# akofke/fountain

Hardware: AMD Instinct MI355X
Metric: Mrays/s (primary+secondary) at fixed spp (higher is better)
Workload: dtype f32; 1 GPU; config 5 scene: 2309 baked copies of rounded_cube = 10002588 triangles (19979703 BVH nodes, depth 29), 4096x4096 film, PathIntegrator(max_depth 5, rr 1.0), 1024^2 env-map light; one step = 16 spp over the whole film; tiles=65536, tiles_per_gpu=65536, pipeline=wavefront, sampler=indexed xoshiro256+, per_gpu_workload=copies=2309,res=4096,spp_per_gpu=16

## Files before the change

fountain_amd/csrc/ftn_device.h:

```cpp
#ifndef FTN_DEVICE_H
#define FTN_DEVICE_H

#include <hip/hip_runtime.h>
#include "ftn_math.h"
#include "../../include/fountain_hip.h"

namespace ftn {

#define FTN_DEV_NOINLINE __device__ inline

#define FTN_GS 3
enum : uint32_t { GF_KIND_SPHERE = 1u, GF_HAS_NORMALS = 2u, GF_HAS_UVS = 4u, GF_FLIP = 8u, GF_LEAF_END = 16u , GF_HAS_TANGENTS = 32u  };
enum : uint32_t { LK_POINT = 0, LK_DISTANT = 1, LK_INFINITE = 2, LK_AREA = 3 };

struct DSphere {
    float o2w[16], o2w_inv[16], w2o[16];
    float radius, z_min, z_max, theta_min, theta_max, phi_max;
    uint32_t reverse_orientation, _pad;
};

struct DLight {
    uint32_t kind; int32_t prim;
    float rgb[3];
    float v[3];
// ... 15 lines not shown

struct DScene {
    const float4* nodes; const float4* geom; const uint4* prim_info;
    uint32_t geom_stride, _pad_gs;
    const float* N; const float* UV;
    const float* T;
    const DSphere* spheres; const ftn_material* materials; const DLight* lights;
    uint32_t n_nodes, n_prims, n_lights, n_inf_lights, n_spheres, _pad;
    const uint32_t* inf_lights;
    const float4* fat;
    float root_lo[3], root_hi[3];
    uint32_t root_is_leaf, n_fat;
    const ftn_texture* textures; const ftn_material_textures* mtex; const DImage* images; const float4* texels;
    uint32_t n_textures;
    uint32_t material_types;
    uint32_t env_only, _pad2;
    DLight env0;
    const float4* srec;
    const float4* quad;
    uint32_t n_quads, quad_stack_bound;
    const uint4* oct; const float4* oct_xbox;
    uint32_t n_octs, oct_stack_bound;
    const uint4* quad64; const float4* quad64_xbox;
    uint32_t n_quad64, quad64_stack_bound;
    const unsigned char* prim_class;
};

struct DCamera {
    float c2w[16]; float r2c[16];
    float shutter_open, shutter_close, lens_radius, focal_dist;
    float dx_camera[3], dy_camera[3];
// ... 906 lines not shown
```

fountain_amd/csrc/ftn_gbuffer.hip:

```cpp
#include "ftn_wf_internal.h"
#include "ftn_texture.h"
#include "ftn_gbuffer.h"
#include <algorithm>
#include <cstring>

namespace ftn {

#define GB_MAX_PASS_THROUGH 4096u
struct GbParams {
    float w2c[16];
    float* out;
    float4 *spillA, *spillB, *spillC;
    float4* rec;
};

__device__ inline Rgb gb_albedo(const ftn_material& m) {
    const Rgb a(m.a[0], m.a[1], m.a[2]), b(m.b[0], m.b[1], m.b[2]);
    switch (m.type) {
        case FTN_MAT_MATTE: return clamp_positive(a);
        case FTN_MAT_MIRROR: return clamp_positive(a);
        case FTN_MAT_METAL: return fresnel_conductor(1.0f, Rgb(1.0f), a, b);
        case FTN_MAT_PLASTIC: return a + b;
        default: return clamp_positive(a) + clamp_positive(b);
    }
// ... 147 lines not shown

int wavefront_gbuffer(WavefrontState** state, const RenderParams& P, const std::vector<DTile>& tiles, const float w2c[16], float* d_out,
                      float4* spill_a, float4* spill_b, float4* spill_c, hipStream_t stream, double* trace_ms_out) {
    knobs_begin();
    { int rc0 = wf_state_init(state); if (rc0) return rc0; }
    WavefrontState* st = *state;
    const uint32_t n_slots = (uint32_t)tiles.size() * 256u;
    const uint32_t total_samples = P.last_sample - P.first_sample;
    if (n_slots == 0 || total_samples == 0) return FTN_OK;
    WfPassPlan plan;
    int rc = wf_plan_passes(st, P, tiles.size() * 256u, total_samples, false, &plan);
    if (rc) return rc;
    const uint32_t S = plan.samples;
    if ((rc = trace4_prepare(st, P.S))) return rc;
    WfBuffers W = st->W;
    W.br = nullptr; W.pd = nullptr; W.pd_md = 0; W.pd_occ = 0; W.drain_sig = nullptr; W.drain_seq = 0; W.serial = 0; W.rng_replay = 0; W.mis_any = 0;
    W.gen_blocks = knob("FTN_GEN_BLOCKS", 1);
    uint32_t valid = 0; for (const DTile& t : tiles) valid += (uint32_t)((t.x1 - t.x0) * (t.y1 - t.y0));
    W.valid_per_sample = valid;
    GbParams G;
    memcpy(G.w2c, w2c, sizeof(G.w2c)); G.out = d_out; G.spillA = spill_a; G.spillB = spill_b; G.spillC = spill_c; G.rec = st->pd;
    const bool spheres = P.S.n_spheres != 0, tex = P.S.n_textures != 0;
    const size_t lds = (size_t)P.stack_entries * 256 * sizeof(uint32_t);
    const unsigned blocks_per_cu = (unsigned)std::max<size_t>(1, std::min<size_t>(8, (size_t)(160 * 1024) / std::max<size_t>(lds, 1)));
    const unsigned trace_grid_max = (unsigned)st->n_cu * blocks_per_cu;
    double trace_ms = 0.0;
    for (uint32_t s0 = 0; s0 < total_samples; s0 += S) {
        const uint32_t Sp = std::min(S, total_samples - s0);
        W.n_slots = n_slots; W.samples = Sp; W.n_paths = Sp * n_slots; W.first_sample = P.first_sample + s0; W.seg_cap = (uint32_t)st->cap_paths;
        launch_wf_new_pass(W, P.stats, stream);
        launch_wf_generate(P, W, 0, stream);
// ... 36 lines not shown
```

fountain_amd/csrc/ftn_scene_host.cpp:

```cpp
#include "ftn_bvh_host.h"
#include "ftn_texture.h"

#include <chrono>
#include <cstdio>
#include <cstdlib>
#include <cstring>
#include <memory>

using namespace ftn;

static Aabb prim_bounds(const ftn_scene_desc* d, const ftn_prim& p) {
    Aabb b = aabb_empty();
    if (p.shape_kind == FTN_SHAPE_TRIANGLE) {
        for (int k = 0; k < 3; k++) { uint32_t v = d->tri_indices[3 * (size_t)p.shape_index + k]; aabb_join_point(b, V3(d->P[3 * v], d->P[3 * v + 1], d->P[3 * v + 2])); }
    } else {
        const ftn_sphere& s = d->spheres[p.shape_index];
        const float lo[3] = {-s.radius, -s.radius, s.z_min}, hi[3] = {s.radius, s.radius, s.z_max};
        for (int c = 0; c < 8; c++) {
            V3 q((c & 4) ? hi[0] : lo[0], (c & 2) ? hi[1] : lo[1], (c & 1) ? hi[2] : lo[2]);
            aabb_join_point(b, m4_point(s.object_to_world.m, q));
        }
    }
    return b;
}
// ... 133 lines not shown
    bool quad64_off = env_is("FTN_QUAD64", 0);
    bool oct_off = env_is("FTN_OCT", 0);
    bool srec_off = env_is("FTN_SREC", 0);
    bool geom_on = env_is("FTN_GEOM", 1);
    bool legacy_arrays_on = env_is("FTN_LEGACY_ARRAYS", 1);
    bool env_cells_off = env_is("FTN_ENV_CELLS", 0);
    bool no_coarse_cdf = getenv("FTN_NO_COARSE_CDF") != nullptr;
    bool want_fat() const { return trace4_off || quad_off || fat_on; }
};

struct Upload {
    const ftn_scene_desc* d; ftn_scene* sc; const HostScene& hs; const SceneKnobs& knobs; size_t np;
    std::vector<float4> geom; std::vector<uint4> info; std::vector<uint8_t> leaf_end;
    std::vector<ftn_material> mats; std::vector<DLight> lights; std::vector<uint32_t> inf;
    uint32_t n_fat = 0, n_quads = 0, quad_bound = 0, n_quad64 = 0, quad64_bound = 0, n_octs = 0, oct_bound = 0;
    bool geom_in_srec = false, has_tex = false;
    Upload(const ftn_scene_desc* d_, ftn_scene* sc_, const SceneKnobs& k) : d(d_), sc(sc_), hs(sc_->host), knobs(k), np(sc_->host.order.size()) {}
};

template <class T> static int held_table(std::vector<DevBuf<T>>& held, const T* src, size_t n, const T** p) {
    held.emplace_back();
    const int rc = held.back().upload(src, n);
    *p = held.back().p;
    return rc;
}

static int node_records(const Upload& U, std::vector<float4>* out) {
    const HostScene& hs = U.hs;
    std::vector<float4>& nodes = *out;
    nodes.resize(2 * hs.nodes.size());
    parallel_for(hs.nodes.size(), [&](size_t i0, size_t i1) { for (size_t i = i0; i < i1; i++) {
// ... 148 lines not shown
    }
    if ((rc = sc->spheres.upload(sph.data(), sph.size()))) return rc;
    U.mats.assign(d->materials, d->materials + d->n_materials);
    U.has_tex = d->n_textures != 0 && d->textures != nullptr;
    for (size_t i = 0; i < U.mats.size(); i++) {
        bool textured = false;
        if (U.has_tex && d->material_textures) { const ftn_material_textures& mt = d->material_textures[i]; textured = (mt.a & mt.b & mt.s0 & mt.s1 & mt.s2) >= 0; }
        if (!textured) material_finalize(U.mats[i]);
    }
    return sc->materials.upload(U.mats.data(), U.mats.size());
}

static int prim_classes(Upload& U) {
    std::vector<unsigned char> cls(U.np);
    for (size_t i = 0; i < U.np; i++) { const int m = (int)U.info[2 * i].x; cls[i] = (unsigned char)(m < 0 || (size_t)m >= U.mats.size() ? 7u : std::min<uint32_t>(2u + U.mats[(size_t)m].type, 7u)); }
    return U.sc->prim_class.upload(cls.data(), cls.size());
}

struct EnvTables { std::vector<float4> tex4; std::vector<float> img, ccdf, cint, mcdf; uint32_t nu = 0, nv = 0; };

static void env_distribution(const ftn_envmap& e, DLight& L, EnvTables* T) {
    const uint32_t height = e.width, width = e.height;
    T->tex4.resize((size_t)e.width * e.height);
    for (size_t k = 0; k < T->tex4.size(); k++) T->tex4[k] = make_float4(e.texels[3 * k], e.texels[3 * k + 1], e.texels[3 * k + 2], 0.0f);
    DLight hostL = L; hostL.texels = T->tex4.data();
    std::vector<float>& img = T->img;
    img.resize((size_t)width * height);
    for (uint32_t j = 0; j < height; j++) {
        float v = (float)j / (float)height;
        float sin_theta = ftn_det::sinf_det(FTN_PI * ((float)j + 0.5f) / (float)height);
// ... 91 lines not shown
        if (L.kind == LK_INFINITE) {
            U.inf.push_back((uint32_t)l);
            if ((rc = env_light_tables(U, src, L))) return rc;
        }
    }
    if ((rc = U.sc->lights.upload(lights.data(), lights.size()))) return rc;
    return U.sc->inf_lights.upload(U.inf.data(), U.inf.size());
}

static void fill_dscene(Upload& U) {
    ftn_scene* sc = U.sc; const HostScene& hs = U.hs;
    DScene& D = sc->d; memset(&D, 0, sizeof(D));
    D.nodes = sc->nodes.p; D.geom = U.geom_in_srec ? sc->srec.p : sc->geom.p; D.geom_stride = U.geom_in_srec ? 8u : (uint32_t)FTN_GS; D.prim_info = sc->prim_info.p; D.N = sc->N.p; D.UV = sc->UV.p; D.T = sc->T.p; D.spheres = sc->spheres.p;
    D.materials = sc->materials.p; D.lights = sc->lights.p; D.inf_lights = sc->inf_lights.p;
    D.n_nodes = (uint32_t)hs.nodes.size(); D.n_prims = (uint32_t)U.np; D.n_lights = (uint32_t)U.lights.size(); D.n_inf_lights = (uint32_t)U.inf.size(); D.n_spheres = U.d->n_spheres;
    D.srec = sc->srec.p; D.prim_class = sc->prim_class.p;
    D.quad = sc->quad.p; D.n_quads = U.n_quads; D.quad_stack_bound = U.quad_bound;
    D.oct = sc->oct.p; D.oct_xbox = sc->oct_xbox.p; D.n_octs = U.n_octs; D.oct_stack_bound = U.oct_bound;
    D.quad64 = sc->quad64.p; D.quad64_xbox = sc->quad64_xbox.p; D.n_quad64 = U.n_quad64; D.quad64_stack_bound = U.quad64_bound;
    D.fat = sc->fat.p; D.n_fat = U.n_fat; D.root_is_leaf = (!hs.nodes.empty() && hs.nodes[0].is_leaf) ? 1u : 0u;
    for (int k = 0; k < 3; k++) { D.root_lo[k] = hs.nodes.empty() ? 0.0f : hs.nodes[0].bmin[k]; D.root_hi[k] = hs.nodes.empty() ? 0.0f : hs.nodes[0].bmax[k]; }
    if (U.lights.size() == 1 && U.lights[0].kind == LK_INFINITE) { D.env_only = 1; D.env0 = U.lights[0]; }
    sc->stack_entries = std::max<uint32_t>(hs.max_depth, 1u);
    for (const ftn_material& m : U.mats) if (m.type < 32u) D.material_types |= 1u << m.type;
}

static int textures_and_pyramids(Upload& U) {
    const ftn_scene_desc* d = U.d; ftn_scene* sc = U.sc;
    if (!U.has_tex) return FTN_OK;
    const int nt = (int)d->n_textures, ni = d->images ? (int)d->n_images : 0;
    std::vector<ftn_material_textures> mt(d->n_materials);
// ... 122 lines not shown
```

fountain_amd/csrc/ftn_wavefront.hip:

```cpp
#include "ftn_wf_internal.h"
#include "ftn_texture.h"
#include <string>
#include <cstdlib>
#include <hipcub/hipcub.hpp>

namespace ftn {

__global__ void __launch_bounds__(256) k_wf_generate(RenderParams P, WfBuffers W, int write_state) {
    const uint32_t i = blockIdx.x * 256u + threadIdx.x;
    if (i >= W.n_paths) return;
    const uint32_t slot = i / W.samples, s = i % W.samples;
    const DTile tile = P.tiles[slot >> 8];
    const int px = tile.x0 + (int)(slot & 15u), py = tile.y0 + (int)((slot >> 4) & 15u);
    if (px < tile.x1 && py < tile.y1) {
        Rng rng; rng.seed(indexed_key(P.seed, px, py, W.first_sample + s));
        V2 j = rng.next2();
        V2 p_film((float)px + j.x, (float)py + j.y);
        V2 p_lens = rng.next2();
        float time_u = rng.next();
        DRay ray = camera_ray(P.C, p_film, p_lens, time_u);
        W.ray[2 * (size_t)(i)] = make_float4(ray.o.x, ray.o.y, ray.o.z, 0.0f);
        W.ray[2 * (size_t)(i) + 1] = make_float4(ray.d.x, ray.d.y, ray.d.z, ray.t_max);
        if (write_state) {
            W.beta[i] = make_float4(1.0f, 1.0f, 1.0f, __uint_as_float(PS_ALIVE));
// ... 234 lines not shown
        uint32_t* T = &W.counters[CTR(13) + 4 * ((policy >> 8) & 7u)];
        atomicMax(&T[0], ~t_start); atomicMax(&T[1], ~t_dry); atomicMax(&T[2], t_dry); atomicMax(&T[3], (uint32_t)wall_clock64());
    }
#endif
    if (blockIdx.x == 0 && threadIdx.x == 0) atomicAdd(&stats->rays_any, (unsigned long long)count);
}

#define WF_NCLASS 8
__device__ inline uint32_t wf_class_of(const RenderParams& P, const WfBuffers& W, uint32_t entry) {
    if (entry & WF_Q_FIN) return 0u;
    const int prim = W.hit_prim[entry & WF_Q_ID_MASK];
    if (prim < 0 || (entry & WF_Q_DEPTH)) return 1u;
    return P.S.prim_class[prim];
}
#define WF_CLS_ROUNDS 32
__global__ void __launch_bounds__(256) k_wf_classify(RenderParams P, WfBuffers W, int in_q) {
    __shared__ unsigned char s_cls[WF_CLS_ROUNDS][256];
    __shared__ uint32_t s_cnt[WF_CLS_ROUNDS][WF_NCLASS][4];
    __shared__ uint32_t s_pre[WF_CLS_ROUNDS][WF_NCLASS];
    __shared__ uint32_t s_base[WF_NCLASS];
    const uint32_t count = W.counters[CTR(in_q == 0 ? 0 : 1)];
    const uint32_t stride = gridDim.x * 256u, rounds = (count + stride - 1) / stride;
    const uint32_t wave = threadIdx.x >> 6, lane = lane_id();
    for (uint32_t r0 = 0; r0 < rounds; r0 += WF_CLS_ROUNDS) {
        const uint32_t nr = rounds - r0 < WF_CLS_ROUNDS ? rounds - r0 : WF_CLS_ROUNDS;
        for (uint32_t r = 0; r < nr; r++) {
            const uint32_t qi = (r0 + r) * stride + blockIdx.x * 256u + threadIdx.x;
            uint32_t c = WF_NCLASS;
            if (qi < count) c = wf_class_of(P, W, W.q_active[in_q][qi]);
            s_cls[r][threadIdx.x] = (unsigned char)c;
#pragma unroll
            for (int k = 0; k < WF_NCLASS; k++) {
                const unsigned long long m = __ballot(c == (uint32_t)k);
                if (lane == 0) s_cnt[r][k][wave] = (uint32_t)__popcll(m);
            }
        }
        __syncthreads();
        if (threadIdx.x < WF_NCLASS) {
            const uint32_t k = threadIdx.x; uint32_t tot = 0;
            for (uint32_t r = 0; r < nr; r++) { s_pre[r][k] = tot; tot += s_cnt[r][k][0] + s_cnt[r][k][1] + s_cnt[r][k][2] + s_cnt[r][k][3]; }
            s_base[k] = tot ? atomicAdd(&W.cls[CTR(k)], tot) : 0u;
        }
        __syncthreads();
        for (uint32_t r = 0; r < nr; r++) {
// ... 12 lines not shown
    }
}

#ifndef FTN_SHADE_MIN_WAVES
#define FTN_SHADE_MIN_WAVES 1
#endif
#ifndef FTN_SHADE_WAVES_NOBSDF
#define FTN_SHADE_WAVES_NOBSDF 4
#endif
#ifndef FTN_SHADE_WAVES_MATTE
#define FTN_SHADE_WAVES_MATTE 3
#endif
#ifndef FTN_SHADE_WAVES_OTHER
#define FTN_SHADE_WAVES_OTHER 3
#endif
template <bool TEX, int MT, bool ENV>
__global__ void __launch_bounds__(256, (MT == -1 ? FTN_SHADE_MIN_WAVES : (MT == -2 ? FTN_SHADE_WAVES_NOBSDF : (MT == 0 ? FTN_SHADE_WAVES_MATTE : FTN_SHADE_WAVES_OTHER)))) k_wf_shade(RenderParams P, WfBuffers W, int in_q, uint32_t class_mask, uint32_t first ) {
    const DScene& S = P.S;
    uint32_t cbase[WF_NCLASS + 1], ccnt[WF_NCLASS];
    cbase[0] = 0;
#pragma unroll
    for (int k = 0; k < WF_NCLASS; k++) { ccnt[k] = ((class_mask >> k) & 1u) ? W.cls[CTR(k)] : 0u; cbase[k + 1] = cbase[k] + ((ccnt[k] + 255u) & ~255u); }
    const uint32_t count = cbase[WF_NCLASS];
    uint32_t* out_q = W.q_active[in_q ^ 1];
    uint32_t* out_count = &W.counters[CTR(in_q == 0 ? 1 : 0)];
    int err = 0;
    const uint32_t stride = gridDim.x * 256u;
    const uint32_t rounds = (count + stride - 1) / stride;
    for (uint32_t round = 0; round < rounds; round++) {
        const uint32_t qi = round * stride + blockIdx.x * 256u + threadIdx.x;
// ... 6 lines not shown
            have = qi - cb < cc;
            sorted_idx = c * W.seg_cap + (qi - cb);
        }
        bool push_active = false, push_closest = false, push_mis = false, push_shadow = false, push_mis_any = false;
        uint32_t p = 0, active_entry = 0;
        if (have) {
            p = W.q_sorted[sorted_idx];
            float4 bq = make_float4(1.0f, 1.0f, 1.0f, __uint_as_float(PS_ALIVE)), lq = make_float4(0.0f, 0.0f, 0.0f, 0.0f);
            if (!first) { if (W.br) { bq = W.br[2 * (size_t)p]; lq = W.br[2 * (size_t)p + 1]; } else { bq = W.beta[p]; lq = W.rad[p]; } }
            Rgb beta(bq.x, bq.y, bq.z), L(lq.x, lq.y, lq.z);
            uint32_t ps = __float_as_uint(bq.w);
            if (ps & PS_DIRECT) {
                float4 q0, q1, q2, q3 = make_float4(0.0f, 0.0f, 0.0f, 0.0f);
                if (W.pd) { const float4* Q = W.pd + 4 * (size_t)p; q0 = Q[0]; q1 = Q[1]; q2 = Q[2]; if (W.pd_md) q3 = Q[3]; } else { q0 = W.pend0[p]; q1 = W.pend1[p]; q2 = W.pend2[p]; }
                const uint32_t occ_word = __float_as_uint(q3.w);
                Rgb radiance(0.0f);
                if ((ps & PS_SHADOW) && !(W.pd_occ ? (occ_word & 0xffu) != 0u : W.occluded[p] != 0)) radiance = radiance + Rgb(q0.x, q0.y, q0.z);
                if (ps & PS_MIS_ANY) {
                    const int light_index = (int)__float_as_uint(lq.w);
                    const DLight& Lt = ENV ? S.env0 : S.lights[light_index];
                    const float4 md = W.pd_md ? q3 : W.ray[2 * (size_t)(p + W.n_paths) + 1];
                    Rgb inc(0.0f);
                    if (!(W.pd_occ ? (occ_word & 0xff00u) != 0u : W.occluded[p + W.n_paths] != 0)) inc = light_Le_env(Lt, V3(md.x, md.y, md.z));
                    if (!inc.is_black()) radiance = radiance + Rgb(q1.x, q1.y, q1.z) * inc * q0.w / q1.w;
                } else if (ps & PS_MIS) {
                    const int light_index = (int)__float_as_uint(lq.w);
                    const DLight& Lt = ENV ? S.env0 : S.lights[light_index];
                    const DHit mh = load_hit(W, p + W.n_paths);
                    const float4 mo = W.ray[2 * (size_t)(p + W.n_paths)], md = W.ray[2 * (size_t)(p + W.n_paths) + 1];
                    Rgb inc(0.0f);
                    if (mh.prim >= 0) {
                      if (!ENV) {
                        int h_mat, h_light; prim_mat_light(S, mh.prim, &h_mat, &h_light);
                        if (h_light >= 0 && h_light == light_index) {
                            DRay r0; r0.o = V3(mo.x, mo.y, mo.z); r0.d = V3(md.x, md.y, md.z); r0.t_max = FTN_INF; r0.time = 0.0f;
                            DSI s2; make_interaction(S, mh, r0, &s2);
                            inc = area_Le(Lt, s2.hit.n, -r0.d);
                        }
                      }
                    } else if (ENV || Lt.kind == LK_INFINITE) inc = light_Le_env(Lt, V3(md.x, md.y, md.z));
                    if (!inc.is_black()) radiance = radiance + Rgb(q1.x, q1.y, q1.z) * inc * q0.w / q1.w;
                }
                Rgb direct = Rgb(q2.x, q2.y, q2.z) * ((float)S.n_lights * radiance);
                L = L + direct;
                ps &= ~(PS_DIRECT | PS_SHADOW | PS_MIS | PS_MIS_ANY);
            }
            if (!(ps & PS_ALIVE)) {
                W.rad[p] = make_float4(L.r, L.g, L.b, 0.0f);
            } else {
                DRay ray0; ray0.o = V3(0.0f, 0.0f, 0.0f); ray0.d = V3(0.0f, 0.0f, 1.0f); ray0.t_max = FTN_INF; ray0.time = 0.0f;
                DHit h; h.t = FTN_INF; h.b0 = 0.0f; h.b1 = 0.0f; h.b2 = 0.0f; h.prim = -1;
                bool need_ray = true;
                if (MT == -2 && !first) { h.prim = W.hit_prim[p]; need_ray = h.prim >= 0 || (ps & PS_BOUNCE_MASK) == 0u || (ps & PS_SPECULAR) != 0u; }
                if (need_ray) {
                    const float4 ro = W.ray[2 * (size_t)(p)], rdv = W.ray[2 * (size_t)(p) + 1];
                    ray0.o = V3(ro.x, ro.y, ro.z); ray0.d = V3(rdv.x, rdv.y, rdv.z); ray0.t_max = rdv.w;
                    h = load_hit(W, p);
                }
                const bool hit = h.prim >= 0;
                uint32_t bounces = ps & PS_BOUNCE_MASK;
                const bool specular_bounce = (ps & PS_SPECULAR) != 0;
                DSI si;
                if (hit) make_interaction(S, h, ray0, &si);
                if (bounces == 0 || specular_bounce) {
                    if (hit) {
                        Rgb e(0.0f);
                        if (!ENV && si.light >= 0) e = area_Le(S.lights[si.light], si.hit.n, -ray0.d);
                        L = L + beta * e;
                    } else L = L + beta * (ENV ? Rgb(0.0f) + light_Le_env(S.env0, ray0.d) : scene_env_Le(S, ray0.d));
                }
                bool alive = true;
                uint32_t light_word = 0;
                if (!hit || bounces >= P.max_depth) alive = false;
                else {
                    Rng rng;
                    if (first) {
                        const uint32_t slot = p / W.samples, sidx = p % W.samples;
                        const DTile tile = P.tiles[slot >> 8];
                        rng.seed(indexed_key(P.seed, tile.x0 + (int)(slot & 15u), tile.y0 + (int)((slot >> 4) & 15u), W.first_sample + sidx));
                        (void)rng.next2(); (void)rng.next2(); (void)rng.next();
                    } else if (W.rng_replay) {
                        const uint32_t slot = p / W.samples, sidx = p % W.samples;
                        const DTile tile = P.tiles[slot >> 8];
                        rng.seed(indexed_key(P.seed, tile.x0 + (int)(slot & 15u), tile.y0 + (int)((slot >> 4) & 15u), W.first_sample + sidx));
// ... 92 lines not shown
                                    float q = fmax_(0.05f, 1.0f - beta.max_component());
                                    n_draws += 1u;
                                    if (rng.next() < q) alive = false; else beta = beta / (1.0f - q);
                                }
                                if (alive) {
                                    W.ray[2 * (size_t)(p)] = make_float4(nr.o.x, nr.o.y, nr.o.z, 0.0f); W.ray[2 * (size_t)(p) + 1] = make_float4(nr.d.x, nr.d.y, nr.d.z, nr.t_max);
                                    bounces += 1; push_closest = true;
                                }
                            } else alive = false;
                        }
                    }
                    if (W.rng_replay) ps = (ps & ((1u << PS_DRAWS_SHIFT) - 1u)) | (n_draws << PS_DRAWS_SHIFT);
                    else if (alive || W.serial) { W.rng01[p] = make_ulonglong2(rng.s0, rng.s1); W.rng23[p] = make_ulonglong2(rng.s2, rng.s3); }
                }
                ps = (ps & ~(PS_BOUNCE_MASK | PS_ALIVE)) | (bounces & PS_BOUNCE_MASK) | (alive ? PS_ALIVE : 0u);
                push_active = alive || (ps & PS_DIRECT);
                if (W.br) {
                    if (push_active) { W.br[2 * (size_t)p] = make_float4(beta.r, beta.g, beta.b, __uint_as_float(ps)); W.br[2 * (size_t)p + 1] = make_float4(L.r, L.g, L.b, __uint_as_float(light_word)); }
                    else W.rad[p] = make_float4(L.r, L.g, L.b, 0.0f);
                } else {
                    if (push_active) W.beta[p] = make_float4(beta.r, beta.g, beta.b, __uint_as_float(ps));
                    W.rad[p] = make_float4(L.r, L.g, L.b, __uint_as_float(light_word));
                }
                active_entry = p | (alive ? (bounces >= P.max_depth ? WF_Q_DEPTH : 0u) : WF_Q_FIN);
            }
            if (W.serial && !push_active) W.ser_retired[p] = 1;
        }
        {
            const bool pred[6] = {push_active, push_closest, push_mis, push_shadow, push_mis_any, push_mis_any};
            const uint32_t val[6] = {active_entry, p, p | WF_MIS_BIT, p, p | WF_MIS_BIT, 0u};
            uint32_t* const qs[6] = {out_q, W.q_closest, W.q_closest, W.q_shadow, W.q_shadow, nullptr};
            uint32_t* const cs[6] = {out_count, &W.counters[CTR(2)], &W.counters[CTR(2)], &W.counters[CTR(3)], &W.counters[CTR(3)], &W.counters[CTR(10)]};
            block_push<6>(pred, val, qs, cs);
// ... 259 lines not shown
        stats->camera_samples += (unsigned long long)W.samples * W.valid_per_sample;
    } else if (mode == 1) {
        W.counters[CTR(2)] = 0; W.counters[CTR(3)] = 0; W.counters[CTR(in_q == 0 ? 1 : 0)] = 0; W.counters[CTR(11)] = 0;
        for (int i = 16; i < 32; i++) W.counters[CTR(i)] = 0;
        for (int i = 32; i < 56; i++) W.counters[CTR(i)] = 0;
    } else if (mode == 2) {
        for (int i = 0; i < WF_NCLASS; i++) W.cls[CTR(i)] = 0;
    } else if (mode == 3) {
        for (int i = 0; i < 64; i++) W.counters[CTR(i)] = 0;
    }
}

#define WF_ACC_CHUNK 8u
__global__ void __launch_bounds__(256) k_wf_accumulate(RenderParams P, WfBuffers W) {
    __shared__ float4 s_rad[256 * WF_ACC_CHUNK];
    const uint32_t slot = blockIdx.x * 256u + threadIdx.x;
    uint32_t spill = 0, bc = 0, cam = 0; int err = 0;
    const FilmSlot fs = film_slot(P, W.n_slots, slot);
    const bool valid = fs.valid, in_crop = fs.in_crop; const int px = fs.px, py = fs.py; const size_t ai = fs.ai;
    float4 acc = make_float4(0.0f, 0.0f, 0.0f, 0.0f);
    if (in_crop) acc = P.accA[ai];
    const size_t block_first = (size_t)blockIdx.x * 256u * W.samples;
    for (uint32_t s0 = 0; s0 < W.samples; s0 += WF_ACC_CHUNK) {
        const uint32_t n = W.samples - s0 < WF_ACC_CHUNK ? W.samples - s0 : WF_ACC_CHUNK;
        for (uint32_t e = threadIdx.x; e < 256u * n; e += 256u) {
            const uint32_t sl = e / n, k = e - sl * n;
            const size_t p = block_first + (size_t)sl * W.samples + s0 + k;
            if (p < W.n_paths) s_rad[sl * WF_ACC_CHUNK + k] = W.rad[p];
        }
        __syncthreads();
        if (valid) {
            for (uint32_t k = 0; k < n; k++) {
                const float4 l = s_rad[threadIdx.x * WF_ACC_CHUNK + k];
                Rgb L(l.x, l.y, l.z);
                if (L.has_nans()) err = FTN_ERR_NAN_RADIANCE;
                Rng crng; crng.seed(indexed_key(P.seed, px, py, W.first_sample + s0 + k));
                const V2 j = crng.next2();
                if (film_add(fs.F, P.accA, P.accB, P.accC, V2((float)px + j.x, (float)py + j.y), L, in_crop ? px : FTN_OWN_NONE, py, &acc, &bc) != 1) spill++;
                cam++;
            }
        }
        __syncthreads();
    }
// ... 365 lines not shown
    if (rc) { wf_free(st); return rc; }
    const bool tex = P.S.n_textures != 0;
    if (n_tiles > st->ser_paths || (tex && !st->ser_tex)) {
        for (void*& m : st->ser_mem) { if (m) (void)hipFree(m); m = nullptr; }
        st->ser_paths = 0;
        WF_TRY(hipMalloc(&st->ser_mem[0], (size_t)n_tiles * sizeof(uint2)));
        WF_TRY(hipMalloc(&st->ser_mem[1], (size_t)n_tiles * sizeof(float2)));
        WF_TRY(hipMalloc(&st->ser_mem[2], (size_t)n_tiles));
        if (tex) WF_TRY(hipMalloc(&st->ser_mem[3], 3 * (size_t)n_tiles * sizeof(float4)));
        st->ser_paths = n_tiles; st->ser_tex = tex;
    }
    if ((rc = trace4_prepare(st, P.S))) return rc;
    WfBuffers W = st->W;
    W.serial = 1; W.ser_cursor = (uint2*)st->ser_mem[0]; W.ser_pfilm = (float2*)st->ser_mem[1]; W.ser_retired = (unsigned char*)st->ser_mem[2]; W.dfd = (float4*)st->ser_mem[3];
    W.n_slots = 0; W.samples = 1; W.n_paths = n_tiles; W.first_sample = 0; W.seg_cap = (uint32_t)st->cap_paths; W.valid_per_sample = 0;
    W.gen_blocks = 0; W.rng_replay = 0; W.br = nullptr; W.pd = nullptr; W.pd_md = 0; W.pd_occ = 0;
    const int count_mode = count ? (count_production ? 2 : 1) : 0;
    W.mis_any = ((!count || count_production) && knob("FTN_MIS_ANY", 1)) ? 1u : 0u;
    const bool spheres = P.S.n_spheres != 0;
    const size_t lds = (size_t)P.stack_entries * 256 * sizeof(uint32_t);
    const unsigned blocks_per_cu = (unsigned)std::max<size_t>(1, std::min<size_t>(8, (size_t)(160 * 1024) / std::max<size_t>(lds, 1)));
    const unsigned tg = std::min<unsigned>((unsigned)st->n_cu * blocks_per_cu, (2 * n_tiles + 255) / 256);
    const dim3 pgrid((n_tiles + 255) / 256), sgrid(std::min<unsigned>((unsigned)st->n_cu * 8u, (n_tiles + 255) / 256));
    const bool env = P.S.env_only && knob("FTN_SHADE_ENV", 1);
    hipEvent_t e0 = st->ev[0], e1 = st->ev[1];
    (void)hipEventRecord(e0, stream);
    hipLaunchKernelGGL(k_wf_reset, dim3(1), dim3(64), 0, stream, W, 3, 0, P.stats);
    if (tex) hipLaunchKernelGGL((k_wf_serial_advance<true>), pgrid, dim3(256), 0, stream, P, W, 0, 1); else hipLaunchKernelGGL((k_wf_serial_advance<false>), pgrid, dim3(256), 0, stream, P, W, 0, 1);
    int in_q = 0; unsigned long long rounds = 0, trace_launches = 0;
    if (!st->ser_host) WF_TRY(hipHostMalloc((void**)&st->ser_host, 2 * 16 * 32 * sizeof(uint32_t)));
    int polled_q[2] = {0, 0}; uint32_t* last = st->ser_host;
    const bool side_ok = st->side != nullptr && knob("FTN_WF_OVERLAP", 2) != 0 && getenv("ROCPROF_COUNTER_COLLECTION") == nullptr;
    const uint64_t max_rounds = 256u * (uint64_t)std::max<uint32_t>(P.spp, 1u) * ((uint64_t)P.max_depth + 4u + (1u << 12));
    for (uint64_t it = 0; it < max_rounds; it++) {
        const bool beside = it > 0 && side_ok;
        if (beside) { WF_TRY(hipEventRecord(st->ev_ready, stream)); WF_TRY(hipStreamWaitEvent(st->side, st->ev_ready, 0));
                      launch_trace(st, true, count_mode, spheres, tg, lds, st->side, P, W, W.q_shadow, &W.counters[CTR(3)], &W.counters[CTR(24)], 2 * n_tiles);
                      WF_TRY(hipEventRecord(st->ev_side, st->side)); }
        launch_trace(st, false, count_mode, spheres, tg, lds, stream, P, W, W.q_closest, &W.counters[CTR(2)], &W.counters[CTR(16)], 2 * n_tiles);
        trace_launches++;
        if (it > 0 && !beside) launch_trace(st, true, count_mode, spheres, tg, lds, stream, P, W, W.q_shadow, &W.counters[CTR(3)], &W.counters[CTR(24)], 2 * n_tiles);
        if (beside) WF_TRY(hipStreamWaitEvent(stream, st->ev_side, 0));
        hipLaunchKernelGGL(k_wf_reset, dim3(1), dim3(64), 0, stream, W, 2, in_q, P.stats);
        hipLaunchKernelGGL(k_wf_classify, sgrid, dim3(256), 0, stream, P, W, in_q);
        hipLaunchKernelGGL(k_wf_reset, dim3(1), dim3(64), 0, stream, W, 1, in_q, P.stats);
#define FTN_SH2(T, M, E, mask) hipLaunchKernelGGL((k_wf_shade<T, M, E>), sgrid, dim3(256), 0, stream, P, W, in_q, mask, 0u)
#define FTN_SH(M, mask) do { if (tex) { if (env) FTN_SH2(true, M, true, mask); else FTN_SH2(true, M, false, mask); } \
                             else { if (env) FTN_SH2(false, M, true, mask); else FTN_SH2(false, M, false, mask); } } while (0)
        if (!knob("FTN_SHADE_SPECIALISE", 1)) FTN_SH(-1, 0xffu);
        else {
            FTN_SH(-2, 0x83u);
            if (P.S.material_types & 1u) FTN_SH(0, 1u << 2);
            if (P.S.material_types & 2u) FTN_SH(1, 1u << 3);
            if (P.S.material_types & 4u) FTN_SH(2, 1u << 4);
            if (P.S.material_types & 8u) FTN_SH(3, 1u << 5);
            if (P.S.material_types & 16u) FTN_SH(4, 1u << 6);
        }
#undef FTN_SH2
#undef FTN_SH
// ... 50 lines not shown
    if ((rc = trace4_prepare(st, P.S))) return rc;
    if (dl_mode) { st->W.dlA = (float4*)st->dl_mem[0]; st->W.dlB = (float4*)st->dl_mem[1]; st->W.whT = (float4*)st->dl_mem[2]; st->W.dfd = (float4*)st->dl_mem[7]; }
    WfBuffers W = st->W;
    if (dl_mode) { W.sh = (float4*)st->dl_mem[3]; W.occluded = (unsigned char*)st->dl_mem[4]; W.q_shadow = (uint32_t*)st->dl_mem[5]; W.q_exc_any = (uint32_t*)st->dl_mem[6]; }
    if (!knob("FTN_ENV_CELLS_USE", 1)) P.S.env0.cells = nullptr;
    const bool spheres = P.S.n_spheres != 0;
    uint32_t valid = 0; for (const DTile& t : tiles) valid += (uint32_t)((t.x1 - t.x0) * (t.y1 - t.y0));
    W.valid_per_sample = valid;
    W.mis_any = ((!count || count_production) && knob("FTN_MIS_ANY", 1)) ? 1u : 0u;
    W.rng_replay = (!dl_mode && 5u + 8u * ((uint32_t)P.max_depth + 1u) <= 511u && knob("FTN_RNG_REPLAY", 1)) ? 1u : 0u;
    W.br = (!dl_mode && knob("FTN_WF_BR", 1)) ? st->br : nullptr;
    W.pd = (!dl_mode && knob("FTN_WF_PD", 3)) ? st->pd : nullptr;
    W.pd_md = (W.pd && knob("FTN_WF_PD", 3) >= 2) ? 1u : 0u;
    W.pd_occ = (W.pd && knob("FTN_WF_PD", 3) >= 3) ? 1u : 0u;
    W.gen_blocks = knob("FTN_GEN_BLOCKS", 1);
    const size_t lds = (size_t)P.stack_entries * 256 * sizeof(uint32_t);
    const unsigned blocks_per_cu = (unsigned)std::max<size_t>(1, std::min<size_t>(8, (size_t)(160 * 1024) / std::max<size_t>(lds, 1)));
    const unsigned trace_grid_max = (unsigned)st->n_cu * blocks_per_cu;
    const unsigned shade_grid_max = (unsigned)st->n_cu * 8u;
    double trace_ms = 0.0; unsigned long long trace_launches = 0, mis_any_rays = 0;
    double group_ms[4] = {0.0, 0.0, 0.0, 0.0}; unsigned long long group_n[4] = {0, 0, 0, 0};
    const uint32_t overlap_mode = knob("FTN_WF_OVERLAP", 2);
    const bool drain_gate = knob("FTN_WF_DRAIN_GATE", 1) != 0 && getenv("ROCPROF_COUNTER_COLLECTION") == nullptr;
    const uint32_t sort_bits = knob("FTN_WF_SORT", 0) ? std::min<uint32_t>(std::max<uint32_t>(knob("FTN_WF_SORT_BITS", 7), 1u), 9u) : 0u;
    uint32_t n_active = 0;
    int ev_used = 0;
    struct Span { int a, b, kind; };
    std::vector<Span> spans;
    static const char* const kGroup[4] = {"closest-hit trace", "any-hit trace", "classify + shade", "queue sort"};
    auto flush_events = [&]() -> int {
// ... 44 lines not shown
            trace_launches++;
            if (beside) WF_TRY(hipStreamWaitEvent(st->side, st->ev_ready, 0));
            if (gated) WF_TRY(hipStreamWaitValue32(st->side, st->drain_sig, W.drain_seq, hipStreamWaitValueGte, 0xffffffffu));
            if (it > 0) {
                const unsigned sg = std::min<unsigned>(trace_grid_max, (2 * W.n_paths + 255) / 256);
                hipStream_t as = beside ? st->side : stream;
                const int e = span_begin(as);
                launch_trace(st, true, count_mode, spheres, sg, lds, as, P, W, q_sh, &W.counters[CTR(3)], &W.counters[CTR(24)], 2 * W.n_paths, it == 1 && W.samples >= 4u);
                span_end(e, 1, as);
                if (beside) WF_TRY(hipEventRecord(st->ev_side, st->side));
            }
            {
                const int e_cls = span_begin(stream);
                const unsigned cg = std::min<unsigned>(shade_grid_max, (W.n_paths + 255) / 256);
                hipLaunchKernelGGL(k_wf_reset, dim3(1), dim3(64), 0, stream, W, 2, in_q, P.stats);
                hipLaunchKernelGGL(k_wf_classify, dim3(cg), dim3(256), 0, stream, P, W, in_q);
                span_end(e_cls, 2, stream);
            }
            if (beside) WF_TRY(hipStreamWaitEvent(stream, st->ev_side, 0));
            const int e_shade = span_begin(stream);
            hipLaunchKernelGGL(k_wf_reset, dim3(1), dim3(64), 0, stream, W, 1, in_q, P.stats);
            {
                const dim3 sgrid(std::min<unsigned>(shade_grid_max, (W.n_paths + 255) / 256));
                const bool tex = P.S.n_textures != 0;
                const uint32_t first = it == 0 ? 1u : 0u;
                if (dl_mode) {
                    if (whitted) { if (tex) hipLaunchKernelGGL((k_wf_shade_dl<true, true>), sgrid, dim3(256), 0, stream, P, W, in_q); else hipLaunchKernelGGL((k_wf_shade_dl<true, false>), sgrid, dim3(256), 0, stream, P, W, in_q); }
                    else { if (tex) hipLaunchKernelGGL((k_wf_shade_dl<false, true>), sgrid, dim3(256), 0, stream, P, W, in_q); else hipLaunchKernelGGL((k_wf_shade_dl<false, false>), sgrid, dim3(256), 0, stream, P, W, in_q); }
                } else if (!knob("FTN_SHADE_SPECIALISE", 1)) {
                    if (tex) hipLaunchKernelGGL((k_wf_shade<true, -1, false>), sgrid, dim3(256), 0, stream, P, W, in_q, 0xffu, first);
                    else hipLaunchKernelGGL((k_wf_shade<false, -1, false>), sgrid, dim3(256), 0, stream, P, W, in_q, 0xffu, first);
                } else {
                    const bool env = P.S.env_only && knob("FTN_SHADE_ENV", 1);
                    const unsigned grid_k = knob("FTN_SHADE_GRID", 0), grid_k_nb = knob("FTN_SHADE_GRID_NOBSDF", 0);
#define FTN_SH2(T, M, E, mask) do { const unsigned per_cu = (M) == -2 ? (grid_k_nb ? grid_k_nb : 2u * shade_wgs_per_cu<T, M, E>()) : (grid_k ? grid_k : shade_wgs_per_cu<T, M, E>()); \
                                    hipLaunchKernelGGL((k_wf_shade<T, M, E>), dim3(std::min<unsigned>((unsigned)st->n_cu * per_cu, (W.n_paths + 255) / 256)), dim3(256), 0, stream, P, W, in_q, mask, first); } while (0)
#define FTN_SH(M, mask) do { if (tex) { if (env) FTN_SH2(true, M, true, mask); else FTN_SH2(true, M, false, mask); } \
                             else { if (env) FTN_SH2(false, M, true, mask); else FTN_SH2(false, M, false, mask); } } while (0)
                    FTN_SH(-2, 0x83u);
                    if (P.S.material_types & 1u) FTN_SH(0, 1u << 2);
                    if (P.S.material_types & 2u) FTN_SH(1, 1u << 3);
                    if (P.S.material_types & 4u) FTN_SH(2, 1u << 4);
                    if (P.S.material_types & 8u) FTN_SH(3, 1u << 5);
                    if (P.S.material_types & 16u) FTN_SH(4, 1u << 6);
#undef FTN_SH2
#undef FTN_SH
                }
            }
            span_end(e_shade, 2, stream);
            in_q ^= 1;
            if (sort_bits) {
                WF_TRY(hipMemcpyAsync(st->host_counters, W.counters, 16 * 32 * sizeof(uint32_t), hipMemcpyDeviceToHost, stream));
                WF_TRY(hipStreamSynchronize(stream));
                polled = true;
// ... 7 lines not shown
                const int e_sort = span_begin(stream);
                if ((rc = sort_ray_queue(st, P, W, false, W.q_closest, st->host_counters[CTR(2)], W.q_sorted, k_in, k_out, sort_bits, stream, &q_cl))) return rc;
                if (knob("FTN_WF_SORT_ANY", 0) && (rc = sort_ray_queue(st, P, W, true, W.q_shadow, st->host_counters[CTR(3)], W.q_sorted + 2 * n, k_in, k_out, sort_bits, stream, &q_sh))) return rc;
                span_end(e_sort, 3, stream);
            }
            if (it >= P.max_depth || polled) {
                if (!polled) {
                    WF_TRY(hipMemcpyAsync(st->host_counters, W.counters, 16 * 32 * sizeof(uint32_t), hipMemcpyDeviceToHost, stream));
                    WF_TRY(hipStreamSynchronize(stream));
                }
                if (it >= P.max_depth && count && knob("FTN_WF_DEBUG", 0)) fprintf(stderr, "[wf] wave steps so far: node %u leaf %u; lanes during node steps (x64): idle %u waiting-with-leaf %u\n", st->host_counters[CTR(6)], st->host_counters[CTR(7)], st->host_counters[CTR(8)], st->host_counters[CTR(9)]);
                n_active = st->host_counters[CTR(in_q == 0 ? 0 : 1)];
                if (n_active == 0) break;
            }
        }
        if (W.mis_any) mis_any_rays += st->host_counters[CTR(10)];
        hipLaunchKernelGGL(k_wf_accumulate, dim3((n_slots + 255) / 256), dim3(256), 0, stream, P, W);
        if (hook) hook(hook_ctx, P, W, stream);
    }
    return FTN_OK;
    };
    rc = render_passes();
    { const int rc_flush = flush_events(); if (!rc) rc = rc_flush; }
    if (rc) return rc;
    WF_TRY(hipGetLastError());
    if (times) {
        times->trace_ms = trace_ms; times->trace_launches = trace_launches; times->mis_any_rays = mis_any_rays;
        times->any_ms = group_ms[1]; times->any_launches = group_n[1]; times->shade_ms = group_ms[2]; times->shade_launches = group_n[2]; times->sort_ms = group_ms[3];
    }
    return FTN_OK;
// ... 4 lines not shown
```

fountain_amd/csrc/ftn_wf_common.h:

```cpp
#ifndef FTN_WF_COMMON_H
#define FTN_WF_COMMON_H
#include "ftn_wavefront.h"
#include "ftn_film.h"

namespace ftn {

enum : uint32_t { PS_BOUNCE_MASK = 0xffffu, PS_SPECULAR = 1u << 16, PS_ALIVE = 1u << 17, PS_DIRECT = 1u << 18, PS_SHADOW = 1u << 19, PS_MIS = 1u << 20, PS_DELTA = 1u << 21, PS_MIS_ANY = 1u << 22  };
#define PS_DRAWS_SHIFT 23
#define WF_MIS_BIT 0x80000000u

struct WfBuffers {
    uint32_t n_paths;
    uint32_t n_slots;
    uint32_t samples;
    uint32_t first_sample;
    float4 *ray;
    float4* hit;
    int* hit_prim;
    float4 *sh;
    unsigned char* occluded;
    float4 *beta;
    float4 *rad;
    float4* br;
    ulonglong2 *rng01, *rng23;
// ... 5 lines not shown
    uint32_t* cls;
    uint32_t seg_cap;
    uint32_t* counters;
    uint32_t valid_per_sample;
    uint32_t* drain_sig; uint32_t drain_seq, drain_at;
    uint32_t *q_exc_closest, *q_exc_any;
    float4 *dlA, *dlB, *whT;
    float4* dfd;
    uint32_t serial;
    uint2* ser_cursor;
    float2* ser_pfilm;
    unsigned char* ser_retired;
    uint32_t rng_replay;
    uint32_t gen_blocks;
    uint32_t mis_any;
};

#define WF_Q_FIN 0x80000000u
#define WF_Q_DEPTH 0x40000000u
#define WF_Q_ID_MASK 0x0fffffffu

#define CTR(i) ((i) * 32)
__device__ inline uint32_t lane_id() { return threadIdx.x & 63u; }
__device__ inline void wave_push(bool pred, uint32_t value, uint32_t* queue, uint32_t* counter) {
    const unsigned long long m = __ballot(pred);
    if (m == 0) return;
    const int leader = __ffsll((long long)m) - 1;
    uint32_t base = 0;
    if ((int)lane_id() == leader) base = atomicAdd(counter, (uint32_t)__popcll(m));
    base = __shfl(base, leader, 64);
// ... 121 lines not shown
```

Baseline: 3234 Mrays/s.

## Defer direct-light and escape finishing to accumulate kernel in env-only wavefront

In env-only scenes with packed path-data buffers, paths no longer re-enter the queue solely to fold in their direct-lighting result. Classification drops hit/escape classes after the first bounce, and the final shadow rays are traced once after the bounce loop. The accumulate kernel then finishes each path by reading beta/L, the pending direct data, hit and ray state, and adding the direct and escaped-env radiance. This removes a shade pass and queue traffic per bounce, but accumulate now does more scattered memory reads per path and the shade path gains conditional buffer writes.

```diff
diff --git a/fountain_amd/csrc/ftn_device.h b/fountain_amd/csrc/ftn_device.h
--- a/fountain_amd/csrc/ftn_device.h
+++ b/fountain_amd/csrc/ftn_device.h
@@ -53,7 +53,8 @@
     const ftn_texture* textures; const ftn_material_textures* mtex; const DImage* images; const float4* texels;
     uint32_t n_textures;
     uint32_t material_types;
-    uint32_t env_only, _pad2;
+    uint32_t env_only;
+    uint32_t null_prims;
     DLight env0;
     const float4* srec;
     const float4* quad;
diff --git a/fountain_amd/csrc/ftn_gbuffer.hip b/fountain_amd/csrc/ftn_gbuffer.hip
--- a/fountain_amd/csrc/ftn_gbuffer.hip
+++ b/fountain_amd/csrc/ftn_gbuffer.hip
@@ -185,7 +185,7 @@
     const uint32_t S = plan.samples;
     if ((rc = trace4_prepare(st, P.S))) return rc;
     WfBuffers W = st->W;
-    W.br = nullptr; W.pd = nullptr; W.pd_md = 0; W.pd_occ = 0; W.drain_sig = nullptr; W.drain_seq = 0; W.serial = 0; W.rng_replay = 0; W.mis_any = 0;
+    W.br = nullptr; W.pd = nullptr; W.pd_md = 0; W.pd_occ = 0; W.drain_sig = nullptr; W.drain_seq = 0; W.serial = 0; W.rng_replay = 0; W.mis_any = 0; W.late_finish = 0;
     W.gen_blocks = knob("FTN_GEN_BLOCKS", 1);
     uint32_t valid = 0; for (const DTile& t : tiles) valid += (uint32_t)((t.x1 - t.x0) * (t.y1 - t.y0));
     W.valid_per_sample = valid;
diff --git a/fountain_amd/csrc/ftn_scene_host.cpp b/fountain_amd/csrc/ftn_scene_host.cpp
--- a/fountain_amd/csrc/ftn_scene_host.cpp
+++ b/fountain_amd/csrc/ftn_scene_host.cpp
@@ -171,7 +171,7 @@
     std::vector<float4> geom; std::vector<uint4> info; std::vector<uint8_t> leaf_end;
     std::vector<ftn_material> mats; std::vector<DLight> lights; std::vector<uint32_t> inf;
     uint32_t n_fat = 0, n_quads = 0, quad_bound = 0, n_quad64 = 0, quad64_bound = 0, n_octs = 0, oct_bound = 0;
-    bool geom_in_srec = false, has_tex = false;
+    bool geom_in_srec = false, has_tex = false, null_prims = false;
     Upload(const ftn_scene_desc* d_, ftn_scene* sc_, const SceneKnobs& k) : d(d_), sc(sc_), hs(sc_->host), knobs(k), np(sc_->host.order.size()) {}
 };
 
@@ -350,6 +350,8 @@
 static int prim_classes(Upload& U) {
     std::vector<unsigned char> cls(U.np);
     for (size_t i = 0; i < U.np; i++) { const int m = (int)U.info[2 * i].x; cls[i] = (unsigned char)(m < 0 || (size_t)m >= U.mats.size() ? 7u : std::min<uint32_t>(2u + U.mats[(size_t)m].type, 7u)); }
+    U.null_prims = false;
+    for (const unsigned char c : cls) if (c == 7u) U.null_prims = true;
     return U.sc->prim_class.upload(cls.data(), cls.size());
 }
 
@@ -471,7 +473,7 @@
     D.nodes = sc->nodes.p; D.geom = U.geom_in_srec ? sc->srec.p : sc->geom.p; D.geom_stride = U.geom_in_srec ? 8u : (uint32_t)FTN_GS; D.prim_info = sc->prim_info.p; D.N = sc->N.p; D.UV = sc->UV.p; D.T = sc->T.p; D.spheres = sc->spheres.p;
     D.materials = sc->materials.p; D.lights = sc->lights.p; D.inf_lights = sc->inf_lights.p;
     D.n_nodes = (uint32_t)hs.nodes.size(); D.n_prims = (uint32_t)U.np; D.n_lights = (uint32_t)U.lights.size(); D.n_inf_lights = (uint32_t)U.inf.size(); D.n_spheres = U.d->n_spheres;
-    D.srec = sc->srec.p; D.prim_class = sc->prim_class.p;
+    D.srec = sc->srec.p; D.prim_class = sc->prim_class.p; D.null_prims = U.null_prims ? 1u : 0u;
     D.quad = sc->quad.p; D.n_quads = U.n_quads; D.quad_stack_bound = U.quad_bound;
     D.oct = sc->oct.p; D.oct_xbox = sc->oct_xbox.p; D.n_octs = U.n_octs; D.oct_stack_bound = U.oct_bound;
     D.quad64 = sc->quad64.p; D.quad64_xbox = sc->quad64_xbox.p; D.n_quad64 = U.n_quad64; D.quad64_stack_bound = U.quad64_bound;
diff --git a/fountain_amd/csrc/ftn_wavefront.hip b/fountain_amd/csrc/ftn_wavefront.hip
--- a/fountain_amd/csrc/ftn_wavefront.hip
+++ b/fountain_amd/csrc/ftn_wavefront.hip
@@ -272,7 +272,7 @@
     return P.S.prim_class[prim];
 }
 #define WF_CLS_ROUNDS 32
-__global__ void __launch_bounds__(256) k_wf_classify(RenderParams P, WfBuffers W, int in_q) {
+__global__ void __launch_bounds__(256) k_wf_classify(RenderParams P, WfBuffers W, int in_q, uint32_t drop ) {
     __shared__ unsigned char s_cls[WF_CLS_ROUNDS][256];
     __shared__ uint32_t s_cnt[WF_CLS_ROUNDS][WF_NCLASS][4];
     __shared__ uint32_t s_pre[WF_CLS_ROUNDS][WF_NCLASS];
@@ -285,7 +285,7 @@
         for (uint32_t r = 0; r < nr; r++) {
             const uint32_t qi = (r0 + r) * stride + blockIdx.x * 256u + threadIdx.x;
             uint32_t c = WF_NCLASS;
-            if (qi < count) c = wf_class_of(P, W, W.q_active[in_q][qi]);
+            if (qi < count) { c = wf_class_of(P, W, W.q_active[in_q][qi]); if ((drop >> c) & 1u) c = WF_NCLASS; }
             s_cls[r][threadIdx.x] = (unsigned char)c;
 #pragma unroll
             for (int k = 0; k < WF_NCLASS; k++) {
@@ -328,6 +328,26 @@
 #ifndef FTN_SHADE_WAVES_OTHER
 #define FTN_SHADE_WAVES_OTHER 3
 #endif
+__device__ inline Rgb wf_add_direct(Rgb L, bool shadow_lit, float4 q0, float4 q1, float4 q2, Rgb inc, uint32_t n_lights) {
+    Rgb radiance(0.0f);
+    if (shadow_lit) radiance = radiance + Rgb(q0.x, q0.y, q0.z);
+    if (!inc.is_black()) radiance = radiance + Rgb(q1.x, q1.y, q1.z) * inc * q0.w / q1.w;
+    Rgb direct = Rgb(q2.x, q2.y, q2.z) * ((float)n_lights * radiance);
+    return L + direct;
+}
+__device__ inline Rgb wf_add_seen(Rgb L, Rgb beta, Rgb e) { return L + beta * e; }
+template <bool ENV> __device__ inline Rgb wf_escaped_Le(const DScene& S, V3 d) { return ENV ? Rgb(0.0f) + light_Le_env(S.env0, d) : scene_env_Le(S, d); }
+__device__ inline Rgb wf_finish_path(const DScene& S, Rgb beta, Rgb L, uint32_t ps, float4 q0, float4 q1, float4 q2, float4 q3, bool hit, V3 d) {
+    if (ps & PS_DIRECT) {
+        const uint32_t occ_word = __float_as_uint(q3.w);
+        Rgb inc(0.0f);
+        if ((ps & PS_MIS_ANY) && !((occ_word & 0xff00u) != 0u)) inc = light_Le_env(S.env0, V3(q3.x, q3.y, q3.z));
+        L = wf_add_direct(L, (ps & PS_SHADOW) && !((occ_word & 0xffu) != 0u), q0, q1, q2, inc, S.n_lights);
+    }
+    if ((ps & PS_ALIVE) && ((ps & PS_BOUNCE_MASK) == 0u || (ps & PS_SPECULAR) != 0u)) L = wf_add_seen(L, beta, hit ? Rgb(0.0f) : wf_escaped_Le<true>(S, d));
+    return L;
+}
+
 template <bool TEX, int MT, bool ENV>
 __global__ void __launch_bounds__(256, (MT == -1 ? FTN_SHADE_MIN_WAVES : (MT == -2 ? FTN_SHADE_WAVES_NOBSDF : (MT == 0 ? FTN_SHADE_WAVES_MATTE : FTN_SHADE_WAVES_OTHER)))) k_wf_shade(RenderParams P, WfBuffers W, int in_q, uint32_t class_mask, uint32_t first ) {
     const DScene& S = P.S;
@@ -364,21 +384,18 @@
                 float4 q0, q1, q2, q3 = make_float4(0.0f, 0.0f, 0.0f, 0.0f);
                 if (W.pd) { const float4* Q = W.pd + 4 * (size_t)p; q0 = Q[0]; q1 = Q[1]; q2 = Q[2]; if (W.pd_md) q3 = Q[3]; } else { q0 = W.pend0[p]; q1 = W.pend1[p]; q2 = W.pend2[p]; }
                 const uint32_t occ_word = __float_as_uint(q3.w);
-                Rgb radiance(0.0f);
-                if ((ps & PS_SHADOW) && !(W.pd_occ ? (occ_word & 0xffu) != 0u : W.occluded[p] != 0)) radiance = radiance + Rgb(q0.x, q0.y, q0.z);
+                const bool shadow_lit = (ps & PS_SHADOW) && !(W.pd_occ ? (occ_word & 0xffu) != 0u : W.occluded[p] != 0);
+                Rgb inc(0.0f);
                 if (ps & PS_MIS_ANY) {
                     const int light_index = (int)__float_as_uint(lq.w);
                     const DLight& Lt = ENV ? S.env0 : S.lights[light_index];
                     const float4 md = W.pd_md ? q3 : W.ray[2 * (size_t)(p + W.n_paths) + 1];
-                    Rgb inc(0.0f);
                     if (!(W.pd_occ ? (occ_word & 0xff00u) != 0u : W.occluded[p + W.n_paths] != 0)) inc = light_Le_env(Lt, V3(md.x, md.y, md.z));
-                    if (!inc.is_black()) radiance = radiance + Rgb(q1.x, q1.y, q1.z) * inc * q0.w / q1.w;
                 } else if (ps & PS_MIS) {
                     const int light_index = (int)__float_as_uint(lq.w);
                     const DLight& Lt = ENV ? S.env0 : S.lights[light_index];
                     const DHit mh = load_hit(W, p + W.n_paths);
                     const float4 mo = W.ray[2 * (size_t)(p + W.n_paths)], md = W.ray[2 * (size_t)(p + W.n_paths) + 1];
-                    Rgb inc(0.0f);
                     if (mh.prim >= 0) {
                       if (!ENV) {
                         int h_mat, h_light; prim_mat_light(S, mh.prim, &h_mat, &h_light);
@@ -389,10 +406,8 @@
                         }
                       }
                     } else if (ENV || Lt.kind == LK_INFINITE) inc = light_Le_env(Lt, V3(md.x, md.y, md.z));
-                    if (!inc.is_black()) radiance = radiance + Rgb(q1.x, q1.y, q1.z) * inc * q0.w / q1.w;
                 }
-                Rgb direct = Rgb(q2.x, q2.y, q2.z) * ((float)S.n_lights * radiance);
-                L = L + direct;
+                L = wf_add_direct(L, shadow_lit, q0, q1, q2, inc, S.n_lights);
                 ps &= ~(PS_DIRECT | PS_SHADOW | PS_MIS | PS_MIS_ANY);
             }
             if (!(ps & PS_ALIVE)) {
@@ -416,8 +431,8 @@
                     if (hit) {
                         Rgb e(0.0f);
                         if (!ENV && si.light >= 0) e = area_Le(S.lights[si.light], si.hit.n, -ray0.d);
-                        L = L + beta * e;
-                    } else L = L + beta * (ENV ? Rgb(0.0f) + light_Le_env(S.env0, ray0.d) : scene_env_Le(S, ray0.d));
+                        L = wf_add_seen(L, beta, e);
+                    } else L = wf_add_seen(L, beta, wf_escaped_Le<ENV>(S, ray0.d));
                 }
                 bool alive = true;
                 uint32_t light_word = 0;
@@ -540,9 +555,9 @@
                     else if (alive || W.serial) { W.rng01[p] = make_ulonglong2(rng.s0, rng.s1); W.rng23[p] = make_ulonglong2(rng.s2, rng.s3); }
                 }
                 ps = (ps & ~(PS_BOUNCE_MASK | PS_ALIVE)) | (bounces & PS_BOUNCE_MASK) | (alive ? PS_ALIVE : 0u);
-                push_active = alive || (ps & PS_DIRECT);
+                push_active = alive || (!W.late_finish && (ps & PS_DIRECT));
                 if (W.br) {
-                    if (push_active) { W.br[2 * (size_t)p] = make_float4(beta.r, beta.g, beta.b, __uint_as_float(ps)); W.br[2 * (size_t)p + 1] = make_float4(L.r, L.g, L.b, __uint_as_float(light_word)); }
+                    if (push_active || W.late_finish) {       W.br[2 * (size_t)p] = make_float4(beta.r, beta.g, beta.b, __uint_as_float(ps)); W.br[2 * (size_t)p + 1] = make_float4(L.r, L.g, L.b, __uint_as_float(light_word)); }
                     else W.rad[p] = make_float4(L.r, L.g, L.b, 0.0f);
                 } else {
                     if (push_active) W.beta[p] = make_float4(beta.r, beta.g, beta.b, __uint_as_float(ps));
@@ -832,6 +847,7 @@
 #define WF_ACC_CHUNK 8u
 __global__ void __launch_bounds__(256) k_wf_accumulate(RenderParams P, WfBuffers W) {
     __shared__ float4 s_rad[256 * WF_ACC_CHUNK];
+    __shared__ unsigned char s_valid[256];
     const uint32_t slot = blockIdx.x * 256u + threadIdx.x;
     uint32_t spill = 0, bc = 0, cam = 0; int err = 0;
     const FilmSlot fs = film_slot(P, W.n_slots, slot);
@@ -839,12 +855,30 @@
     float4 acc = make_float4(0.0f, 0.0f, 0.0f, 0.0f);
     if (in_crop) acc = P.accA[ai];
     const size_t block_first = (size_t)blockIdx.x * 256u * W.samples;
+    if (W.late_finish) { s_valid[threadIdx.x] = valid ? 1 : 0; __syncthreads(); }
     for (uint32_t s0 = 0; s0 < W.samples; s0 += WF_ACC_CHUNK) {
         const uint32_t n = W.samples - s0 < WF_ACC_CHUNK ? W.samples - s0 : WF_ACC_CHUNK;
         for (uint32_t e = threadIdx.x; e < 256u * n; e += 256u) {
             const uint32_t sl = e / n, k = e - sl * n;
             const size_t p = block_first + (size_t)sl * W.samples + s0 + k;
-            if (p < W.n_paths) s_rad[sl * WF_ACC_CHUNK + k] = W.rad[p];
+            if (p >= W.n_paths) continue;
+            if (!W.late_finish) { s_rad[sl * WF_ACC_CHUNK + k] = W.rad[p]; continue; }
+            float4 r = make_float4(0.0f, 0.0f, 0.0f, 0.0f);
+            if (s_valid[sl]) {
+                const float4 bq = W.br[2 * p], lq = W.br[2 * p + 1];
+                const uint32_t ps = __float_as_uint(bq.w);
+                float4 q0 = r, q1 = r, q2 = r, q3 = r;
+                if (ps & PS_DIRECT) { const float4* Q = W.pd + 4 * p; q0 = Q[0]; q1 = Q[1]; q2 = Q[2]; q3 = Q[3]; }
+                bool hit = false; V3 d(0.0f, 0.0f, 1.0f);
+                if (ps & PS_ALIVE) {
+                    hit = W.hit_prim[p] >= 0;
+                    if (!hit && ((ps & PS_BOUNCE_MASK) == 0u || (ps & PS_SPECULAR) != 0u)) { const float4 rdv = W.ray[2 * p + 1]; d = V3(rdv.x, rdv.y, rdv.z); }
+                }
+                const Rgb L = wf_finish_path(P.S, Rgb(bq.x, bq.y, bq.z), Rgb(lq.x, lq.y, lq.z), ps, q0, q1, q2, q3, hit, d);
+                r = make_float4(L.r, L.g, L.b, 0.0f);
+            }
+            if (W.late_finish == 2u) W.rad[p] = r;
+            s_rad[sl * WF_ACC_CHUNK + k] = r;
         }
         __syncthreads();
         if (valid) {
@@ -1240,7 +1274,7 @@
     WfBuffers W = st->W;
     W.serial = 1; W.ser_cursor = (uint2*)st->ser_mem[0]; W.ser_pfilm = (float2*)st->ser_mem[1]; W.ser_retired = (unsigned char*)st->ser_mem[2]; W.dfd = (float4*)st->ser_mem[3];
     W.n_slots = 0; W.samples = 1; W.n_paths = n_tiles; W.first_sample = 0; W.seg_cap = (uint32_t)st->cap_paths; W.valid_per_sample = 0;
-    W.gen_blocks = 0; W.rng_replay = 0; W.br = nullptr; W.pd = nullptr; W.pd_md = 0; W.pd_occ = 0;
+    W.gen_blocks = 0; W.rng_replay = 0; W.br = nullptr; W.pd = nullptr; W.pd_md = 0; W.pd_occ = 0; W.late_finish = 0;
     const int count_mode = count ? (count_production ? 2 : 1) : 0;
     W.mis_any = ((!count || count_production) && knob("FTN_MIS_ANY", 1)) ? 1u : 0u;
     const bool spheres = P.S.n_spheres != 0;
@@ -1268,7 +1302,7 @@
         if (it > 0 && !beside) launch_trace(st, true, count_mode, spheres, tg, lds, stream, P, W, W.q_shadow, &W.counters[CTR(3)], &W.counters[CTR(24)], 2 * n_tiles);
         if (beside) WF_TRY(hipStreamWaitEvent(stream, st->ev_side, 0));
         hipLaunchKernelGGL(k_wf_reset, dim3(1), dim3(64), 0, stream, W, 2, in_q, P.stats);
-        hipLaunchKernelGGL(k_wf_classify, sgrid, dim3(256), 0, stream, P, W, in_q);
+        hipLaunchKernelGGL(k_wf_classify, sgrid, dim3(256), 0, stream, P, W, in_q, 0u);
         hipLaunchKernelGGL(k_wf_reset, dim3(1), dim3(64), 0, stream, W, 1, in_q, P.stats);
 #define FTN_SH2(T, M, E, mask) hipLaunchKernelGGL((k_wf_shade<T, M, E>), sgrid, dim3(256), 0, stream, P, W, in_q, mask, 0u)
 #define FTN_SH(M, mask) do { if (tex) { if (env) FTN_SH2(true, M, true, mask); else FTN_SH2(true, M, false, mask); } \
@@ -1349,6 +1383,8 @@
     W.pd_md = (W.pd && knob("FTN_WF_PD", 3) >= 2) ? 1u : 0u;
     W.pd_occ = (W.pd && knob("FTN_WF_PD", 3) >= 3) ? 1u : 0u;
     W.gen_blocks = knob("FTN_GEN_BLOCKS", 1);
+    W.late_finish = (!dl_mode && W.br && W.pd && W.pd_md && W.pd_occ && W.mis_any && P.S.env_only && knob("FTN_SHADE_ENV", 1) && knob("FTN_SHADE_SPECIALISE", 1) &&
+                     knob("FTN_WF_LATE_FINISH", 1)) ? (hook ? 2u : 1u) : 0u;
     const size_t lds = (size_t)P.stack_entries * 256 * sizeof(uint32_t);
     const unsigned blocks_per_cu = (unsigned)std::max<size_t>(1, std::min<size_t>(8, (size_t)(160 * 1024) / std::max<size_t>(lds, 1)));
     const unsigned trace_grid_max = (unsigned)st->n_cu * blocks_per_cu;
@@ -1423,7 +1459,7 @@
                 const int e_cls = span_begin(stream);
                 const unsigned cg = std::min<unsigned>(shade_grid_max, (W.n_paths + 255) / 256);
                 hipLaunchKernelGGL(k_wf_reset, dim3(1), dim3(64), 0, stream, W, 2, in_q, P.stats);
-                hipLaunchKernelGGL(k_wf_classify, dim3(cg), dim3(256), 0, stream, P, W, in_q);
+                hipLaunchKernelGGL(k_wf_classify, dim3(cg), dim3(256), 0, stream, P, W, in_q, (W.late_finish && it > 0) ? 0x3u : 0u);
                 span_end(e_cls, 2, stream);
             }
             if (beside) WF_TRY(hipStreamWaitEvent(stream, st->ev_side, 0));
@@ -1446,7 +1482,8 @@
                                     hipLaunchKernelGGL((k_wf_shade<T, M, E>), dim3(std::min<unsigned>((unsigned)st->n_cu * per_cu, (W.n_paths + 255) / 256)), dim3(256), 0, stream, P, W, in_q, mask, first); } while (0)
 #define FTN_SH(M, mask) do { if (tex) { if (env) FTN_SH2(true, M, true, mask); else FTN_SH2(true, M, false, mask); } \
                              else { if (env) FTN_SH2(false, M, true, mask); else FTN_SH2(false, M, false, mask); } } while (0)
-                    FTN_SH(-2, 0x83u);
+                    if (!W.late_finish || first) FTN_SH(-2, 0x83u);
+                    else if (P.S.null_prims) FTN_SH(-2, 0x80u);
                     if (P.S.material_types & 1u) FTN_SH(0, 1u << 2);
                     if (P.S.material_types & 2u) FTN_SH(1, 1u << 3);
                     if (P.S.material_types & 4u) FTN_SH(2, 1u << 4);
@@ -1484,6 +1521,12 @@
                 if (n_active == 0) break;
             }
         }
+        if (W.late_finish && st->host_counters[CTR(3)] != 0) {
+            if (ev_used + 2 > 64) { rc = flush_events(); if (rc) return rc; }
+            const int e = span_begin(stream);
+            launch_trace(st, true, count_mode, spheres, std::min<unsigned>(trace_grid_max, (2 * W.n_paths + 255) / 256), lds, stream, P, W, q_sh, &W.counters[CTR(3)], &W.counters[CTR(24)], 2 * W.n_paths, false);
+            span_end(e, 1, stream);
+        }
         if (W.mis_any) mis_any_rays += st->host_counters[CTR(10)];
         hipLaunchKernelGGL(k_wf_accumulate, dim3((n_slots + 255) / 256), dim3(256), 0, stream, P, W);
         if (hook) hook(hook_ctx, P, W, stream);
diff --git a/fountain_amd/csrc/ftn_wf_common.h b/fountain_amd/csrc/ftn_wf_common.h
--- a/fountain_amd/csrc/ftn_wf_common.h
+++ b/fountain_amd/csrc/ftn_wf_common.h
@@ -43,6 +43,7 @@
     uint32_t rng_replay;
     uint32_t gen_blocks;
     uint32_t mis_any;
+    uint32_t late_finish;
 };
 
 #define WF_Q_FIN 0x80000000u
```

Result: faster. 3346 Mrays/s, median of 6 (+3.5%).
